# luchsonice/3dod

Measured on AMD Instinct MI355X. Metric: images/sec Cube R-CNN DLA34-FPN train step, higher is better.
Workload: dtype fp32; 1 GPU; Cube R-CNN DLA34+FPN train step (fwd+loss+bwd+allreduce+SGD), 4 img/GPU 512x512, Base_Omni3D.yaml semantics (BASELINE configs[3] per-GPU shard); global_batch=4, parallelism=dp1, weight_gradient_reduce=pixel splits stored and added in a fixed order (CR_DETERMINISTIC=1), valid=True

## Files before the change

3dod_amd/_lib.py:

```python
import ctypes
import os
import threading

import torch

_HERE = os.path.dirname(os.path.abspath(__file__))
LIB_PATH = os.path.join(_HERE, "lib", "libcr3dod.so")

c_void_p, c_int, c_int64, c_float = ctypes.c_void_p, ctypes.c_int, ctypes.c_int64, ctypes.c_float
P = c_void_p

SIGNATURES = {
    "cr_ctx_create": [c_int, P, ctypes.POINTER(P)],
    "cr_ctx_destroy": [P],
    "cr_ctx_set_stream": [P, P],
    "cr_abi_version": [],
    "cr_cuboid_corners": [P, P, P, c_int64, P],
    "cr_cubes_project_score": [P, P, c_int64, c_int64, P, c_int, c_float, c_float, P, P, P, P,
                               P, P, P, P, P, P, P, P, P],
    "cr_cubes_project_score_fast": [P, P, c_int64, c_int64, P, c_int, c_float, c_float, P, P, P, P,
                                    P, P, P, P, P, P, P, P, P, P],
    "cr_propose": [P, P, c_int64, P, c_int, c_int, P, P, P, c_int64, P, c_int, P, P, P, P, P],
    "cr_ransac_plane": [P, P, c_int64, P, c_int64, c_float, P, P, P],
    "cr_ransac_plane_batched": [P, P, P, c_int, c_int64, P, c_int64, c_float, P, P, P],
# ... 10 lines not shown
    "cr_scale_residual_layernorm": [P, P, P, P, P, P, P, P, c_int64, c_int, c_float],
    "cr_scale_residual": [P, P, P, P, P, c_int64, c_int],
    "cr_resize_bilinear_ac": [P, P, P, c_int, c_int, c_int, c_int, c_int, c_int],
    "cr_conv2d_fwd": [P, P, P, P, c_int, c_int, c_int, c_int, c_int, c_int, c_int, c_int, P, P, c_int, P, c_int, c_int, P],
    "cr_conv2d_bwd_data": [P, P, P, P, c_int, c_int, c_int, c_int, c_int, c_int, c_int, c_int, c_int, P, P],
    "cr_weight_split3": [P, P, P, c_int64, c_int],
    "cr_relu_bwd": [P, P, P, P, c_int64, c_int],
    "cr_gt_pack": [P, P, P, P, P, P, c_int, c_int, P, P, P, P],
    "cr_rpn_unpack": [P, P, P, c_int, c_int, c_int, c_int, P, P, P],
    "cr_rpn_pack_grad": [P, P, P, P, P, c_int, c_int, c_int, c_int],
    "cr_topk_blocks": [c_int64, c_int],
    "cr_topk": [P, P, c_int, c_int64, c_int, P, P, P],
    "cr_multi_seg": [P, P, c_int, c_int64, c_int],
    "cr_loss_guard": [P, P, c_int, c_float, P, P, P, c_int, c_float, c_float, P],
    "cr_step_counters": [P, P, P, P],
    "cr_weights_split3": [P, P, P, P, c_int, c_int64],
    "cr_conv2d_bwd_weight": [P, P, P, P, c_int, c_int, c_int, c_int, c_int, c_int, c_int, c_int, c_int, c_int],
    "cr_conv2d_bwd_weight_bias": [P, P, P, P, P, c_int, c_int, c_int, c_int, c_int, c_int, c_int, c_int, c_int, c_int],
    "cr_cast_f32_to_bf16": [P, P, P, c_int64],
    "cr_weight_transpose": [P, P, P, c_int, c_int, c_int, c_int],
    "cr_colsum_accum": [P, P, c_int, c_int64, c_int, P, P],
    "cr_bn_fwd": [P, P, P, c_int, P, P, P, P, c_int64, c_int, c_int, c_float, c_float, P, P, P, c_int],
    "cr_bn_bwd": [P, P, P, P, P, P, P, P, P, P, P, c_int64, c_int, c_int, c_int],
    "cr_bn_frozen_unfold": [P, P, P, P, P, P, P, c_float, P, c_int, P, P, c_int, c_int],
    "cr_pool2x_fwd": [P, P, P, c_int, c_int, c_int, c_int, c_int, c_int],
    "cr_pool2x_bwd": [P, P, P, P, c_int, c_int, c_int, c_int, c_int, c_int, P],
    "cr_upsample2x_add": [P, P, P, P, c_int, c_int, c_int, c_int, c_int],
    "cr_sum2x2": [P, P, P, c_int, c_int, c_int, c_int, c_int],
    "cr_preprocess": [P, P, P, c_int, c_int, c_int, P, P, c_int],
    "cr_roi_align_fwd": [P, P, P, P, P, c_int, c_int, P, c_int64, c_int, c_int, P, c_int],
    "cr_roi_align_bwd": [P, P, P, P, P, c_int, c_int, P, c_int64, c_int, c_int, P, c_int],
    "cr_conv2d_fwd_group": [P, c_int, P, P, P, P, P, P, c_int, c_int, c_int, c_int, P, P, c_int, c_int],
    "cr_wino_filter": [P, P, P, c_int, c_int, c_int],
    "cr_gemm_batched_f32": [P, P, P, P, c_int, c_int, c_int, c_int, c_int64, c_int64, c_int64],
    "cr_wino_input": [P, c_int, P, P, P, P, c_int, P, c_int64],
    "cr_wino_output": [P, c_int, P, P, P, P, P, c_int, c_int64, P, c_int, P],
    "cr_wino_dy": [P, c_int, P, P, P, P, c_int, P, c_int64, P],
    "cr_wino_filter_grad": [P, P, P, c_int, c_int, P, P],
    "cr_wgrad_batched_f32": [P, P, P, P, c_int, c_int, c_int, c_int, c_int64, c_int64, c_int64],
    "cr_conv2d_bwd_data_group": [P, c_int, P, P, P, P, P, P, c_int, c_int, c_int, c_int, c_int, P],
    "cr_conv2d_bwd_weight_group": [P, c_int, P, P, P, P, P, P, P, c_int, c_int, c_int, c_int, c_int],
    "cr_conv2d_bwd_weight_multi": [P, c_int, P, P, P, P, P, P, P, P, P, P, P, P, c_int],
    "cr_roi_align_bwd_set": [P, P, P, P, P, c_int, c_int, c_int, P, c_int64, c_int, c_int, P, c_int],
    "cr_nms_grouped": [P, P, P, c_int, c_int, c_float, P, P],
    "cr_cube_loss_fwd": [P, P, c_int64, c_int, c_int, c_int, c_int, P, P],
    "cr_cube_loss_bwd": [P, P, c_int64, c_int, c_int, c_int, c_int, P, P, P, P, P, P],
# ... 133 lines not shown
```

3dod_amd/csrc/conv.hip:

```cpp
#include "cr_common.h"
#include "cr_elem.h"
#include <stdlib.h>
#include <type_traits>

typedef __bf16 bf16x8 __attribute__((ext_vector_type(8)));
typedef __bf16 bf16x4 __attribute__((ext_vector_type(4)));
typedef short s16x4 __attribute__((ext_vector_type(4)));
typedef float f32x4 __attribute__((ext_vector_type(4)));

#define CONV_T 256

struct ConvP {
    const void* x;
    const void* w;
    void* y;
    const void* res;
    const float* bias;
    float* stats;
    int N, Hin, Win, Cin, Hout, Wout, Cout;
    int stride, pad, Kdim, M, cshift, relu;
    unsigned x_bytes, w_bytes;
    int f32;
    float* part;
    int ksplit, kstages;
// ... 3039 lines not shown

extern "C" int cr_fc_grad_accum(cr_ctx* ctx, const void* g, float* acc, int O, int C, int HW, int act_f32) {
    CR_CHECK_ARG(ctx && g && acc && O > 0 && C > 0 && HW > 0 && HW <= 1024, "cr_fc_grad_accum: bad args");
    if (HW == 1) {
        const int64_t n = (int64_t)O * C;
        CR_CHECK_ARG((((uintptr_t)g) & 7) == 0 && (((uintptr_t)acc) & 15) == 0, "cr_fc_grad_accum: misaligned");
        if (act_f32)
            hipLaunchKernelGGL(k_axpy_f32_f32, dim3((unsigned)cr_cdiv(cr_cdiv(n, 4), 256)), dim3(256), 0, ctx->stream,
                               (const float*)g, acc, n);
        else
            hipLaunchKernelGGL(k_axpy_bf16_f32, dim3((unsigned)cr_cdiv(cr_cdiv(n, 4), 256)), dim3(256), 0, ctx->stream,
                               (const u16*)g, acc, n);
    } else if (act_f32) {
        hipLaunchKernelGGL(k_fc_grad_accum<float>, dim3((unsigned)cr_cdiv(C, FC_CT), O), dim3(256),
                           FC_CT * (HW + 1) * sizeof(float), ctx->stream, (const float*)g, acc, C, HW);
    } else {
        hipLaunchKernelGGL(k_fc_grad_accum<u16>, dim3((unsigned)cr_cdiv(C, FC_CT), O), dim3(256),
                           FC_CT * (HW + 1) * sizeof(float), ctx->stream, (const u16*)g, acc, C, HW);
    }
    CR_LAUNCH_CHECK();
    return CR_OK;
}

__global__ __launch_bounds__(256) void k_bn_finalize(const float* __restrict__ stats, int nparts, int C, float count,
                                                     float eps, float momentum, float* __restrict__ mean_invstd,
                                                     float* __restrict__ running_mean, float* __restrict__ running_var) {
    __shared__ double ss[256], sq[256];
    const int c = blockIdx.x, t = threadIdx.x;
    double s = 0.0, q = 0.0;
    for (int r = t; r < nparts; r += 256) {
        s += (double)stats[(size_t)r * 2 * C + c];
        q += (double)stats[(size_t)r * 2 * C + C + c];
    }
    ss[t] = s; sq[t] = q;
    __syncthreads();
    for (int off = 128; off > 0; off >>= 1) {
        if (t < off) { ss[t] += ss[t + off]; sq[t] += sq[t + off]; }
        __syncthreads();
    }
    if (t == 0) {
        const double mean = ss[0] / (double)count;
        double var = sq[0] / (double)count - mean * mean;
        if (var < 0.0) var = 0.0;
        mean_invstd[c] = (float)mean;
        mean_invstd[C + c] = (float)(1.0 / sqrt(var + (double)eps));
        if (running_mean) {
            const double unbiased = count > 1.f ? var * (double)count / ((double)count - 1.0) : var;
            running_mean[c] = (float)((1.0 - momentum) * running_mean[c] + momentum * mean);
            running_var[c] = (float)((1.0 - momentum) * running_var[c] + momentum * unbiased);
        }
    }
}

template <typename T>
__global__ __launch_bounds__(256) void k_bn_apply(const T* __restrict__ x, const float* __restrict__ mean_invstd,
                                                  const float* __restrict__ gamma, const float* __restrict__ beta,
                                                  const T* __restrict__ res, T* __restrict__ y, int64_t M, int C,
                                                  int relu) {
    const int cg = C >> 3;
    const int64_t total = M * cg;
    for (int64_t i = (int64_t)blockIdx.x * blockDim.x + threadIdx.x; i < total; i += (int64_t)gridDim.x * blockDim.x) {
        const int c0 = (int)(i % cg) << 3;
        float xv[8], rv[8], o[8];
        load8<T>(x, (size_t)i * 8, xv);
        if (res) load8<T>(res, (size_t)i * 8, rv);
#pragma unroll
        for (int e = 0; e < 8; ++e) {
            const int c = c0 + e;
            float t = (xv[e] - mean_invstd[c]) * mean_invstd[C + c] * gamma[c] + beta[c];
            if (res) t += rv[e];
            o[e] = relu ? fmaxf(t, 0.f) : t;
        }
        store8<T>(y, (size_t)i * 8, o);
    }
}

template <typename T>
__global__ __launch_bounds__(256) void k_bn_apply_fused(const T* __restrict__ x, const float* __restrict__ stats, int nparts,
                                                        float count, float eps, float momentum, float* __restrict__ mean_invstd,
                                                        float* __restrict__ running_mean, float* __restrict__ running_var,
                                                        const float* __restrict__ gamma, const float* __restrict__ beta,
                                                        const T* __restrict__ res, T* __restrict__ y, int64_t M, int C, int relu,
                                                        int px_per_block) {
    __shared__ double sd[2][8][32];
    __shared__ float sc[2][32];
    const int t = threadIdx.x, ch = t & 31, rl = t >> 5;
    const int cbase = blockIdx.y * 32, c = cbase + ch;
    {
        double s = 0.0, q = 0.0;
        for (int r = rl; r < nparts; r += 8) {
            s += (double)stats[(size_t)r * 2 * C + c];
            q += (double)stats[(size_t)r * 2 * C + C + c];
// ... 17 lines not shown
            if (running_mean) {
                const double unbiased = count > 1.f ? var * (double)count / ((double)count - 1.0) : var;
                running_mean[cbase + t] = (float)((1.0 - momentum) * running_mean[cbase + t] + momentum * mean);
                running_var[cbase + t] = (float)((1.0 - momentum) * running_var[cbase + t] + momentum * unbiased);
            }
        }
    }
    __syncthreads();
    const int cgl = t & 3;
    float mu[8], is8[8], ga[8], be[8];
#pragma unroll
    for (int e = 0; e < 8; ++e) {
        mu[e] = sc[0][cgl * 8 + e]; is8[e] = sc[1][cgl * 8 + e];
        ga[e] = gamma[cbase + cgl * 8 + e]; be[e] = beta[cbase + cgl * 8 + e];
    }
    const int64_t m0 = (int64_t)blockIdx.x * px_per_block, m1 = m0 + px_per_block < M ? m0 + px_per_block : M;
    for (int64_t m = m0 + (t >> 2); m < m1; m += 64) {
        const size_t i8 = (size_t)m * C + cbase + cgl * 8;
        float xv[8], rv[8], o[8];
        load8<T>(x, i8, xv);
        if (res) load8<T>(res, i8, rv);
#pragma unroll
        for (int e = 0; e < 8; ++e) {
            float v = (xv[e] - mu[e]) * is8[e] * ga[e] + be[e];
            if (res) v += rv[e];
            o[e] = relu ? fmaxf(v, 0.f) : v;
        }
        store8<T>(y, i8, o);
    }
}

static constexpr int BN_FUSE_ROWS = 256;

extern "C" int cr_bn_fwd(cr_ctx* ctx, const void* x, const float* stats, int nparts, const float* gamma,
                         const float* beta, const void* residual, void* y, int64_t M, int C, int relu, float eps,
                         float momentum, float* mean_invstd, float* running_mean, float* running_var, int act_f32) {
    CR_CHECK_ARG(ctx && x && stats && gamma && beta && y && mean_invstd, "cr_bn_fwd: NULL pointer");
    CR_CHECK_ARG(M > 0 && C > 0 && C % 8 == 0 && nparts > 0, "cr_bn_fwd: bad dims M=%lld C=%d", (long long)M, C);
    if (C % 32 == 0 && nparts <= BN_FUSE_ROWS) {
        int64_t chunks = 1024 / (C / 32);
        if (chunks < 1) chunks = 1;
        int64_t ppb = cr_cdiv(M, chunks);
        ppb = (ppb + 63) / 64 * 64;
        const dim3 grid((unsigned)cr_cdiv(M, ppb), (unsigned)(C / 32));
        if (act_f32)
            hipLaunchKernelGGL(k_bn_apply_fused<float>, grid, dim3(256), 0, ctx->stream, (const float*)x, stats, nparts, (float)M,
                               eps, momentum, mean_invstd, running_mean, running_var, gamma, beta, (const float*)residual,
                               (float*)y, M, C, relu, (int)ppb);
        else
            hipLaunchKernelGGL(k_bn_apply_fused<u16>, grid, dim3(256), 0, ctx->stream, (const u16*)x, stats, nparts, (float)M,
                               eps, momentum, mean_invstd, running_mean, running_var, gamma, beta, (const u16*)residual,
                               (u16*)y, M, C, relu, (int)ppb);
        CR_LAUNCH_CHECK();
        return CR_OK;
    }
    hipLaunchKernelGGL(k_bn_finalize, dim3((unsigned)C), dim3(256), 0, ctx->stream, stats, nparts, C, (float)M, eps,
                       momentum, mean_invstd, running_mean, running_var);
    CR_LAUNCH_CHECK();
    const int64_t total = M * (C >> 3);
    const unsigned grid = (unsigned)(cr_cdiv(total, 256) < 4096 ? cr_cdiv(total, 256) : 4096);
    if (act_f32)
        hipLaunchKernelGGL(k_bn_apply<float>, dim3(grid), dim3(256), 0, ctx->stream, (const float*)x, mean_invstd, gamma, beta,
                           (const float*)residual, (float*)y, M, C, relu);
    else
        hipLaunchKernelGGL(k_bn_apply<u16>, dim3(grid), dim3(256), 0, ctx->stream, (const u16*)x, mean_invstd, gamma, beta,
                           (const u16*)residual, (u16*)y, M, C, relu);
    CR_LAUNCH_CHECK();
    return CR_OK;
}

#define BNB_MAXBLOCKS 1024
template <typename T>
__global__ __launch_bounds__(256) void k_bn_bwd_reduce(const T* __restrict__ dy, const T* __restrict__ out,
                                                       const T* __restrict__ x, const float* __restrict__ mean_invstd,
                                                       float* __restrict__ partial, int64_t M, int C, int relu) {
    extern __shared__ float s_acc[];
    const int cg = C >> 3;
    const int mycg = threadIdx.x % cg, myrow = threadIdx.x / cg;
    const int rows_per_block = blockDim.x / cg;
    const int c0 = mycg << 3;
    float a[8], b[8], mu[8], is[8];
#pragma unroll
    for (int e = 0; e < 8; ++e) { a[e] = 0.f; b[e] = 0.f; mu[e] = mean_invstd[c0 + e]; is[e] = mean_invstd[C + c0 + e]; }
    for (int64_t m = (int64_t)blockIdx.x * rows_per_block + myrow; m < M; m += (int64_t)gridDim.x * rows_per_block) {
        const size_t i8 = (size_t)(m * cg + mycg) * 8;
        float dv[8], xv[8], ov[8];
        load8<T>(dy, i8, dv);
        load8<T>(x, i8, xv);
        if (relu) load8<T>(out, i8, ov);
#pragma unroll
        for (int e = 0; e < 8; ++e) {
            const float gq = (!relu || ov[e] > 0.f) ? dv[e] : 0.f;
            const float xh = (xv[e] - mu[e]) * is[e];
            a[e] += gq;
            b[e] += gq * xh;
        }
    }
#pragma unroll
    for (int e = 0; e < 8; ++e) { s_acc[(myrow * 2 + 0) * C + c0 + e] = a[e]; s_acc[(myrow * 2 + 1) * C + c0 + e] = b[e]; }
    __syncthreads();
    float* dst = partial + (size_t)blockIdx.x * 2 * C;
    for (int i = threadIdx.x; i < 2 * C; i += blockDim.x) {
        const int which = i / C, c = i - which * C;
        float s = 0.f;
        for (int r = 0; r < rows_per_block; ++r) s += s_acc[(r * 2 + which) * C + c];
        dst[i] = s;
    }
}

__global__ __launch_bounds__(256) void k_bn_bwd_finalize(const float* __restrict__ partial, int nparts, int C,
                                                         float* __restrict__ sums, float* __restrict__ dgamma,
                                                         float* __restrict__ dbeta) {
    __shared__ double ss[256], sq[256];
    const int c = blockIdx.x, t = threadIdx.x;
    double s = 0.0, q = 0.0;
    for (int r = t; r < nparts; r += 256) {
        s += (double)partial[(size_t)r * 2 * C + c];
        q += (double)partial[(size_t)r * 2 * C + C + c];
    }
    ss[t] = s; sq[t] = q;
    __syncthreads();
    for (int off = 128; off > 0; off >>= 1) {
        if (t < off) { ss[t] += ss[t + off]; sq[t] += sq[t + off]; }
        __syncthreads();
    }
    if (t == 0) {
        sums[c] = (float)ss[0];
        sums[C + c] = (float)sq[0];
        dbeta[c] += (float)ss[0];
        dgamma[c] += (float)sq[0];
    }
}

template <typename T>
__global__ __launch_bounds__(256) void k_bn_bwd_apply(const T* __restrict__ dy, const T* __restrict__ out,
                                                      const T* __restrict__ x, const float* __restrict__ mean_invstd,
                                                      const float* __restrict__ gamma, const float* __restrict__ sums,
                                                      T* __restrict__ dx, T* __restrict__ dres, int64_t M, int C,
                                                      int relu) {
    const int cg = C >> 3;
    const float invM = 1.f / (float)M;
    const int64_t total = M * cg;
    for (int64_t i = (int64_t)blockIdx.x * blockDim.x + threadIdx.x; i < total; i += (int64_t)gridDim.x * blockDim.x) {
        const int c0 = (int)(i % cg) << 3;
        const size_t i8 = (size_t)i * 8;
        float dv[8], xv[8], ov[8], vd[8], vg[8];
        load8<T>(dy, i8, dv);
        load8<T>(x, i8, xv);
        if (relu) load8<T>(out, i8, ov);
#pragma unroll
        for (int e = 0; e < 8; ++e) {
            const int c = c0 + e;
            const float gq = (!relu || ov[e] > 0.f) ? dv[e] : 0.f;
            const float is = mean_invstd[C + c];
            const float xh = (xv[e] - mean_invstd[c]) * is;
            vd[e] = gamma[c] * is * (gq - sums[c] * invM - xh * sums[C + c] * invM);
            vg[e] = gq;
        }
        store8<T>(dx, i8, vd);
        if (dres) store8<T>(dres, i8, vg);
    }
}

template <typename T>
__global__ __launch_bounds__(256) void k_bn_bwd_apply_fused(const T* __restrict__ dy, const T* __restrict__ out,
                                                            const T* __restrict__ x, const float* __restrict__ mean_invstd,
                                                            const float* __restrict__ gamma, const float* __restrict__ partial,
                                                            int nparts, T* __restrict__ dx, T* __restrict__ dres,
                                                            float* __restrict__ dgamma, float* __restrict__ dbeta, int64_t M,
                                                            int C, int relu, int px_per_block) {
    __shared__ double sd[2][8][32];
    __shared__ float sc[4][32];
    const int t = threadIdx.x, ch = t & 31, rl = t >> 5;
    const int cbase = blockIdx.y * 32, c = cbase + ch;
    {
        double s = 0.0, q = 0.0;
        for (int r = rl; r < nparts; r += 8) {
            s += (double)partial[(size_t)r * 2 * C + c];
            q += (double)partial[(size_t)r * 2 * C + C + c];
        }
        sd[0][rl][ch] = s; sd[1][rl][ch] = q;
    }
    __syncthreads();
    if (t < 32) {
        double s = 0.0, q = 0.0;
#pragma unroll
        for (int r = 0; r < 8; ++r) { s += sd[0][r][t]; q += sd[1][r][t]; }
        const float sg = (float)s, sgx = (float)q, invM = 1.f / (float)M;
        const float is = mean_invstd[C + cbase + t];
        sc[0][t] = mean_invstd[cbase + t];
        sc[1][t] = is;
        sc[2][t] = sg * invM;
        sc[3][t] = sgx * invM;
        if (blockIdx.x == 0) { dbeta[cbase + t] += sg; dgamma[cbase + t] += sgx; }
    }
    __syncthreads();
    const int cgl = t & 3;
    float mu[8], is8[8], ga[8], k1[8], k2[8];
#pragma unroll
    for (int e = 0; e < 8; ++e) {
        const int cc = cgl * 8 + e;
        mu[e] = sc[0][cc]; is8[e] = sc[1][cc]; ga[e] = gamma[cbase + cc]; k1[e] = sc[2][cc]; k2[e] = sc[3][cc];
    }
    const int64_t m0 = (int64_t)blockIdx.x * px_per_block, m1 = m0 + px_per_block < M ? m0 + px_per_block : M;
    for (int64_t m = m0 + (t >> 2); m < m1; m += 64) {
        const size_t i8 = (size_t)m * C + cbase + cgl * 8;
        float dv[8], xv[8], ov[8], vd[8], vg[8];
        load8<T>(dy, i8, dv);
        load8<T>(x, i8, xv);
        if (relu) load8<T>(out, i8, ov);
#pragma unroll
        for (int e = 0; e < 8; ++e) {
            const float gq = (!relu || ov[e] > 0.f) ? dv[e] : 0.f;
            const float xh = (xv[e] - mu[e]) * is8[e];
            vd[e] = ga[e] * is8[e] * (gq - k1[e] - xh * k2[e]);
            vg[e] = gq;
        }
        store8<T>(dx, i8, vd);
        if (dres) store8<T>(dres, i8, vg);
    }
}

extern "C" int cr_bn_bwd(cr_ctx* ctx, const void* dy, const void* out, const void* x, const float* mean_invstd,
                         const float* gamma, float* sums, void* dx, void* dres, float* dgamma, float* dbeta,
                         int64_t M, int C, int relu, int act_f32) {
    CR_CHECK_ARG(ctx && dy && x && mean_invstd && gamma && sums && dx && dgamma && dbeta, "cr_bn_bwd: NULL pointer");
    CR_CHECK_ARG(!relu || out, "cr_bn_bwd: relu needs the forward output");
    CR_CHECK_ARG(M > 0 && C % 8 == 0 && C <= 2048 && 256 % (C >> 3) == 0, "cr_bn_bwd: unsupported C=%d", C);
    const int rows_per_block = 256 / (C >> 3);
    int64_t nb = cr_cdiv(M, (int64_t)rows_per_block * 8);
    if (nb > BNB_MAXBLOCKS) nb = BNB_MAXBLOCKS;
    if (nb < 1) nb = 1;
    float* reduced = sums + (size_t)BNB_MAXBLOCKS * 2 * C;
    const size_t shm = sizeof(float) * rows_per_block * 2 * C;
    if (act_f32)
        hipLaunchKernelGGL(k_bn_bwd_reduce<float>, dim3((unsigned)nb), dim3(256), shm, ctx->stream, (const float*)dy,
                           (const float*)out, (const float*)x, mean_invstd, sums, M, C, relu);
    else
        hipLaunchKernelGGL(k_bn_bwd_reduce<u16>, dim3((unsigned)nb), dim3(256), shm, ctx->stream, (const u16*)dy,
                           (const u16*)out, (const u16*)x, mean_invstd, sums, M, C, relu);
    CR_LAUNCH_CHECK();
    if (C % 32 == 0 && nb <= BN_FUSE_ROWS) {
        int64_t chunks = 1024 / (C / 32);
        if (chunks < 1) chunks = 1;
        int64_t ppb = cr_cdiv(M, chunks);
        ppb = (ppb + 63) / 64 * 64;
        const dim3 grid((unsigned)cr_cdiv(M, ppb), (unsigned)(C / 32));
        if (act_f32)
            hipLaunchKernelGGL(k_bn_bwd_apply_fused<float>, grid, dim3(256), 0, ctx->stream, (const float*)dy, (const float*)out,
                               (const float*)x, mean_invstd, gamma, sums, (int)nb, (float*)dx, (float*)dres, dgamma, dbeta, M, C,
                               relu, (int)ppb);
        else
            hipLaunchKernelGGL(k_bn_bwd_apply_fused<u16>, grid, dim3(256), 0, ctx->stream, (const u16*)dy, (const u16*)out,
                               (const u16*)x, mean_invstd, gamma, sums, (int)nb, (u16*)dx, (u16*)dres, dgamma, dbeta, M, C, relu,
                               (int)ppb);
        CR_LAUNCH_CHECK();
        return CR_OK;
    }
    hipLaunchKernelGGL(k_bn_bwd_finalize, dim3((unsigned)C), dim3(256), 0, ctx->stream, sums, (int)nb, C, reduced, dgamma,
                       dbeta);
    CR_LAUNCH_CHECK();
    const int64_t total = M * (C >> 3);
    const unsigned grid = (unsigned)(cr_cdiv(total, 256) < 4096 ? cr_cdiv(total, 256) : 4096);
    if (act_f32)
        hipLaunchKernelGGL(k_bn_bwd_apply<float>, dim3(grid), dim3(256), 0, ctx->stream, (const float*)dy, (const float*)out,
                           (const float*)x, mean_invstd, gamma, reduced, (float*)dx, (float*)dres, M, C, relu);
    else
        hipLaunchKernelGGL(k_bn_bwd_apply<u16>, dim3(grid), dim3(256), 0, ctx->stream, (const u16*)dy, (const u16*)out,
                           (const u16*)x, mean_invstd, gamma, reduced, (u16*)dx, (u16*)dres, M, C, relu);
    CR_LAUNCH_CHECK();
    return CR_OK;
}

template <typename T>
__global__ __launch_bounds__(256) void k_colsum_partial(const T* __restrict__ x, int64_t M, int C, int rows_per_block,
                                                        float* __restrict__ partial) {
    const int64_t r0 = (int64_t)blockIdx.x * rows_per_block;
    const int64_t r1 = r0 + rows_per_block < M ? r0 + rows_per_block : M;
    for (int c = threadIdx.x; c < C; c += 256) {
        float s = 0.f;
        for (int64_t r = r0; r < r1; ++r) {
            if (sizeof(T) == 2) s += bf2f(((const u16*)x)[r * C + c]);
            else s += ((const float*)x)[r * C + c];
        }
        partial[(size_t)blockIdx.x * C + c] = s;
    }
}

__global__ __launch_bounds__(256) void k_colsum_final(const float* __restrict__ partial, int nparts, int C,
                                                      float* __restrict__ out) {
    __shared__ double ss[256];
    const int c = blockIdx.x, t = threadIdx.x;
    double s = 0.0;
    for (int r = t; r < nparts; r += 256) s += (double)partial[(size_t)r * C + c];
// ... 399 lines not shown
```

3dod_amd/csrc/cr_elem.h:

```cpp
#pragma once
#include <hip/hip_runtime.h>

typedef unsigned short u16;

__device__ __forceinline__ float bf2f(u16 b) { return __uint_as_float(((unsigned)b) << 16); }
__device__ __forceinline__ u16 f2bf(float f) {
    __bf16 b = (__bf16)f;
    return __builtin_bit_cast(u16, b);
}

__device__ __forceinline__ void unpack8(const uint4 v, float* f) {
    f[0] = bf2f((u16)(v.x & 0xffff)); f[1] = bf2f((u16)(v.x >> 16));
    f[2] = bf2f((u16)(v.y & 0xffff)); f[3] = bf2f((u16)(v.y >> 16));
    f[4] = bf2f((u16)(v.z & 0xffff)); f[5] = bf2f((u16)(v.z >> 16));
    f[6] = bf2f((u16)(v.w & 0xffff)); f[7] = bf2f((u16)(v.w >> 16));
}
__device__ __forceinline__ uint4 pack8(const float* f) {
    uint4 o;
    o.x = (unsigned)f2bf(f[0]) | ((unsigned)f2bf(f[1]) << 16);
    o.y = (unsigned)f2bf(f[2]) | ((unsigned)f2bf(f[3]) << 16);
    o.z = (unsigned)f2bf(f[4]) | ((unsigned)f2bf(f[5]) << 16);
    o.w = (unsigned)f2bf(f[6]) | ((unsigned)f2bf(f[7]) << 16);
    return o;
}

template <typename T> __device__ __forceinline__ void load8(const T* __restrict__ p, size_t e, float* f);
template <> __device__ __forceinline__ void load8<u16>(const u16* __restrict__ p, size_t e, float* f) {
    unpack8(*reinterpret_cast<const uint4*>(p + e), f);
}
template <> __device__ __forceinline__ void load8<float>(const float* __restrict__ p, size_t e, float* f) {
    const float4 a = *reinterpret_cast<const float4*>(p + e), b = *reinterpret_cast<const float4*>(p + e + 4);
    f[0] = a.x; f[1] = a.y; f[2] = a.z; f[3] = a.w; f[4] = b.x; f[5] = b.y; f[6] = b.z; f[7] = b.w;
}
template <typename T> __device__ __forceinline__ void store8(T* __restrict__ p, size_t e, const float* f);
template <> __device__ __forceinline__ void store8<u16>(u16* __restrict__ p, size_t e, const float* f) {
    *reinterpret_cast<uint4*>(p + e) = pack8(f);
}
template <> __device__ __forceinline__ void store8<float>(float* __restrict__ p, size_t e, const float* f) {
    *reinterpret_cast<float4*>(p + e) = make_float4(f[0], f[1], f[2], f[3]);
    *reinterpret_cast<float4*>(p + e + 4) = make_float4(f[4], f[5], f[6], f[7]);
}
template <typename T> __device__ __forceinline__ float load1(const T* __restrict__ p, size_t e);
template <> __device__ __forceinline__ float load1<u16>(const u16* __restrict__ p, size_t e) { return bf2f(p[e]); }
template <> __device__ __forceinline__ float load1<float>(const float* __restrict__ p, size_t e) { return p[e]; }
```

3dod_amd/hipops.py:

```python
import contextlib
import ctypes
import os

import torch

from . import _lib

bf16 = torch.bfloat16
f32 = torch.float32
STAT_REPL = 32

_PRECISIONS = {"fp32": (f32, 1), "f32": (f32, 1), "float32": (f32, 1), "fp32x3": (f32, 2), "bf16": (bf16, 0),
               "bfloat16": (bf16, 0)}
_ACT = [_PRECISIONS[os.environ.get("CR_PRECISION", "fp32").lower()]]


def set_precision(name):
    prev = precision()
    _ACT[0] = _PRECISIONS[str(name).lower()]
    return prev


def precision():
    return {0: "bf16", 1: "fp32", 2: "fp32x3"}[_ACT[0][1]]
# ... 307 lines not shown
            nparts = (M + 63) // 64
            stats = torch.empty((nparts, 2, Cout), dtype=f32, device=dev)
            y_raw = conv_fwd_raw(x, wb, Cout, k, stride, pad, stats=stats)
            out = torch.empty_like(y_raw)
            mi = torch.empty((2, Cout), dtype=f32, device=dev)
            _lib.call("cr_bn_fwd", y_raw, stats, nparts, gamma.detach(), beta.detach(), residual, out, M, Cout, int(relu),
                      float(eps), float(momentum), mi, running_mean, running_var, af)
        else:
            K_ = weight.numel() // Cout
            wf32 = torch.empty((Cout, K_), dtype=f32, device=dev)
            bias_f = torch.empty((Cout,), dtype=f32, device=dev)
            _lib.call("cr_fold_bn", weight.detach(), gamma.detach(), beta.detach(), running_mean, running_var, float(eps), wf32,
                      bias_f, Cout, K_, 1)
            if x.dtype == bf16:
                wf = torch.empty((Cout, K_), dtype=bf16, device=dev)
                _lib.call("cr_cast_f32_to_bf16", wf32, wf, wf32.numel())
            else:
                wf = wf32
            out = conv_fwd_raw(x, wf, Cout, k, stride, pad, bias=bias_f, residual=residual, relu=relu)
            y_raw, mi = wf32, None
            ctx.frozen = (running_mean, running_var, float(eps))
        ctx.cfg = (k, stride, pad, relu, training, residual is not None)
        ctx.beta_ref = beta
        ctx.save_for_backward(x, weight, gamma, y_raw, out if relu else None, mi)
        return out

    @staticmethod
    def backward(ctx, dout):
        return _ConvBN._backward_impl(ctx, dout)

    @staticmethod
    def _backward_impl(ctx, dout, want_dx=None, want_dw=None):
        x, weight, gamma, y_raw, out, mi = ctx.saved_tensors
        k, stride, pad, relu, training, has_res = ctx.cfg
        root = want_dx is not None
        need_dx = ctx.needs_input_grad[0] if want_dx is None else want_dx
        need_dw = ctx.needs_input_grad[1] if want_dw is None else want_dw
        if not training:
            return _ConvBN._frozen_backward(ctx, dout, need_dx, need_dw, root)
        Cout = weight.shape[0]
        dev = x.device
        dout = dout.to(x.dtype).contiguous()
        M = y_raw.numel() // Cout
        sums = torch.empty((1025, 2, Cout), dtype=f32, device=dev)
        dx_raw = torch.empty_like(y_raw)
        dres = torch.empty_like(y_raw) if has_res else None
        gs, bs = grad_sink(gamma), grad_sink(ctx.beta_ref)
        if gs is not None and bs is not None:
            dgamma, dbeta, ret_g, ret_b = gs, bs, None, None
        else:
            dgamma = torch.zeros((Cout,), dtype=f32, device=dev)
            dbeta = torch.zeros((Cout,), dtype=f32, device=dev)
            ret_g, ret_b = dgamma, dbeta
        _lib.call("cr_bn_bwd", dout, out, y_raw, mi, gamma.detach(), sums, dx_raw, dres, dgamma, dbeta, M, Cout, int(relu),
                  _af(x))
        (xslot, xi), (rslot, ri) = ctx.slots
        if rslot is not None and dres is not None:
            _slot_put(rslot, dres)
            dres = None
        dx = None
        if need_dx:
            _, wt = prepared_weights(weight, True, x.dtype)
            if xslot is not None and xi > 1:
                _slot_put(xslot, conv_bwd_data_raw(dx_raw, wt, x.shape, k, stride, pad, accumulate=_slot_fold(xslot)))
            else:
                acc = _slot_take(xslot) if xslot is not None else None
                dx = conv_bwd_data_raw(dx_raw, wt, x.shape, k, stride, pad, accumulate=acc)
        elif xslot is not None:
            raise RuntimeError("gradient slot registered for an input that needs no gradient")
        dw = conv_bwd_weight_raw(dx_raw, x, k, stride, pad, grad_sink(weight)) if need_dw else None
        if root:
            return dx_raw, dw, ret_g, ret_b
        return dx, dw, ret_g, ret_b, dres, None, None, None, None, None, None, None, None, None

    @staticmethod
    def _frozen_backward(ctx, dout, need_dx, need_dw, root):
        x, weight, gamma, wf32, out, _ = ctx.saved_tensors
        k, stride, pad, relu, _, has_res = ctx.cfg
# ... 1701 lines not shown
```

include/cr3dod.h:

```cpp
#ifndef CR3DOD_H
#define CR3DOD_H

#include <stdint.h>

#ifdef __cplusplus
extern "C" {
#endif

typedef struct cr_ctx cr_ctx;

#define CR_OK 0
#define CR_EINVAL (-22)
#define CR_ENOMEM (-12)
#define CR_EHIP (-5)
#define CR_ERANGE (-34)

int cr_ctx_create(int device, void* hip_stream, cr_ctx** out);
int cr_ctx_destroy(cr_ctx* ctx);
int cr_ctx_set_stream(cr_ctx* ctx, void* hip_stream);
const char* cr_last_error(void);
int cr_abi_version(void);


int cr_cuboid_corners(cr_ctx* ctx, const float* box6, const float* R, int64_t n, float* verts);
// ... 99 lines not shown

int cr_conv2d_fwd_group(cr_ctx* ctx, int n, const void* const* xs, const void* const* ws, void* const* ys, const int* Ns,
                        const int* Hs, const int* Ws, int Cin, int Cout, int ks, int pad, const float* const* biases,
                        const void* const* residuals, int relu, int act_f32);
int cr_conv2d_bwd_data_group(cr_ctx* ctx, int n, const void* const* dys, const void* const* wts, void* const* dxs,
                             const int* Ns, const int* Hs, const int* Ws, int Cin, int Cout, int ks, int pad, int act_f32,
                             const void* const* accumulates);
int cr_conv2d_bwd_weight_group(cr_ctx* ctx, int n, const void* const* dys, const void* const* xs, float* const* dws,
                               float* const* dbiases, const int* Ns, const int* Hs, const int* Ws, int Cin, int Cout, int ks,
                               int pad, int act_f32);
int cr_conv2d_bwd_weight_multi(cr_ctx* ctx, int n, const void* const* dys, const void* const* xs, float* const* dws,
                               float* const* dbiases, const int* Ns, const int* Hs, const int* Ws, const int* Cins,
                               const int* Couts, const int* kss, const int* strides, const int* pads, int act_f32);
int cr_cast_f32_to_bf16(cr_ctx* ctx, const float* src, void* dst, int64_t n);
int cr_colsum_accum(cr_ctx* ctx, const void* x, int is_f32, int64_t M, int C, float* ws, float* out);
int cr_weight_transpose(cr_ctx* ctx, const float* w, void* wt, int Cout, int ks, int Cin, int act_f32);

int cr_bn_fwd(cr_ctx* ctx, const void* x, const float* stats, int nparts, const float* gamma, const float* beta,
              const void* residual, void* y, int64_t M, int C, int relu, float eps, float momentum,
              float* mean_invstd, float* running_mean, float* running_var, int act_f32);
int cr_bn_bwd(cr_ctx* ctx, const void* dy, const void* out, const void* x, const float* mean_invstd,
              const float* gamma, float* sums, void* dx, void* dres, float* dgamma, float* dbeta, int64_t M,
              int C, int relu, int act_f32);
int cr_bn_frozen_unfold(cr_ctx* ctx, const float* dwf, const float* sg, const float* w, const float* gamma,
                        const float* mean, const float* var, float eps, float* dw, int accumulate, float* dgamma,
                        float* dbeta, int Cout, int K);

int cr_pool2x_fwd(cr_ctx* ctx, const void* x, void* y, int N, int H, int W, int C, int window, int act_f32);
int cr_pool2x_bwd(cr_ctx* ctx, const void* x, const void* dy, void* dx, int N, int H, int W, int C, int window, int act_f32,
                  const void* accumulate);
int cr_upsample2x_add(cr_ctx* ctx, const void* lat, const void* top, void* y, int N, int H, int W, int C, int act_f32);
int cr_sum2x2(cr_ctx* ctx, const void* dy, void* dtop, int N, int H, int W, int C, int act_f32);
int cr_preprocess(cr_ctx* ctx, const unsigned char* img, void* y, int N, int H, int W, const float* mean3,
                  const float* std3, int act_f32);

int cr_roi_align_fwd(cr_ctx* ctx, const void* const* feats, const int* Hs, const int* Ws, const float* scales,
                     int nlev, int C, const float* rois, int64_t R, int PH, int PW, void* out, int act_f32);
int cr_roi_align_bwd(cr_ctx* ctx, float* const* grads, const int* Hs, const int* Ws, const float* scales,
                     int nlev, int C, const float* rois, int64_t R, int PH, int PW, const void* dout, int act_f32);
int cr_roi_align_bwd_set(cr_ctx* ctx, float* const* grads, const int* Hs, const int* Ws, const float* scales,
                         int nlev, int C, int N, const float* rois, int64_t R, int PH, int PW, const void* dout,
                         int act_f32);
int cr_nms_grouped(cr_ctx* ctx, const float* boxes, const int* counts, int G, int maxn, float thresh,
                   void* mask_ws, unsigned char* keep);

int cr_cube_loss_fwd(cr_ctx* ctx, const float* const* inputs, int64_t n, int allocentric, int chamfer_pose,
// ... 130 lines not shown
```

Measured before the change: 279.3 images/s.

## Recompute BN ReLU mask in backward and parallelize BN stats finalize

```diff
diff --git a/3dod_amd/_lib.py b/3dod_amd/_lib.py
--- a/3dod_amd/_lib.py
+++ b/3dod_amd/_lib.py
@@ -56,6 +56,7 @@
     "cr_colsum_accum": [P, P, c_int, c_int64, c_int, P, P],
     "cr_bn_fwd": [P, P, P, c_int, P, P, P, P, c_int64, c_int, c_int, c_float, c_float, P, P, P, c_int],
     "cr_bn_bwd": [P, P, P, P, P, P, P, P, P, P, P, c_int64, c_int, c_int, c_int],
+    "cr_bn_bwd_mask": [P, P, P, P, P, P, P, P, P, P, P, P, c_int64, c_int, c_int, c_int],
     "cr_bn_frozen_unfold": [P, P, P, P, P, P, P, c_float, P, c_int, P, P, c_int, c_int],
     "cr_pool2x_fwd": [P, P, P, c_int, c_int, c_int, c_int, c_int, c_int],
     "cr_pool2x_bwd": [P, P, P, P, c_int, c_int, c_int, c_int, c_int, c_int, P],
diff --git a/3dod_amd/csrc/conv.hip b/3dod_amd/csrc/conv.hip
--- a/3dod_amd/csrc/conv.hip
+++ b/3dod_amd/csrc/conv.hip
@@ -3085,35 +3085,81 @@
     return CR_OK;
 }
 
+__device__ __forceinline__ void bn_finalize_tail(double s, double q, int c, int C, float count, float eps, float momentum,
+                                                 float* __restrict__ mean_invstd, float* __restrict__ running_mean,
+                                                 float* __restrict__ running_var) {
+    __shared__ double ss[256], sq[256];
+    const int t = threadIdx.x;
+    ss[t] = s; sq[t] = q;
+    __syncthreads();
+    for (int off = 128; off > 0; off >>= 1) {
+        if (t < off) { ss[t] += ss[t + off]; sq[t] += sq[t + off]; }
+        __syncthreads();
+    }
+    if (t == 0) {
+#pragma clang fp contract(off)
+        const double mean = ss[0] / (double)count;
+        double var = __builtin_fma(-mean, mean, sq[0] / (double)count);
+        if (var < 0.0) var = 0.0;
+        mean_invstd[c] = (float)mean;
+        mean_invstd[C + c] = (float)(1.0 / sqrt(var + (double)eps));
+        if (running_mean) {
+            const double unbiased = count > 1.f ? var * (double)count / ((double)count - 1.0) : var;
+            running_mean[c] = (float)__builtin_fma((double)momentum, mean, (1.0 - momentum) * running_mean[c]);
+            running_var[c] = (float)__builtin_fma((double)momentum, unbiased, (1.0 - momentum) * running_var[c]);
+        }
+    }
+}
+
 __global__ __launch_bounds__(256) void k_bn_finalize(const float* __restrict__ stats, int nparts, int C, float count,
                                                      float eps, float momentum, float* __restrict__ mean_invstd,
                                                      float* __restrict__ running_mean, float* __restrict__ running_var) {
-    __shared__ double ss[256], sq[256];
     const int c = blockIdx.x, t = threadIdx.x;
     double s = 0.0, q = 0.0;
     for (int r = t; r < nparts; r += 256) {
         s += (double)stats[(size_t)r * 2 * C + c];
         q += (double)stats[(size_t)r * 2 * C + C + c];
     }
-    ss[t] = s; sq[t] = q;
-    __syncthreads();
-    for (int off = 128; off > 0; off >>= 1) {
-        if (t < off) { ss[t] += ss[t + off]; sq[t] += sq[t + off]; }
-        __syncthreads();
-    }
-    if (t == 0) {
-        const double mean = ss[0] / (double)count;
-        double var = sq[0] / (double)count - mean * mean;
-        if (var < 0.0) var = 0.0;
-        mean_invstd[c] = (float)mean;
-        mean_invstd[C + c] = (float)(1.0 / sqrt(var + (double)eps));
-        if (running_mean) {
-            const double unbiased = count > 1.f ? var * (double)count / ((double)count - 1.0) : var;
-            running_mean[c] = (float)((1.0 - momentum) * running_mean[c] + momentum * mean);
-            running_var[c] = (float)((1.0 - momentum) * running_var[c] + momentum * unbiased);
-        }
-    }
-}
+    bn_finalize_tail(s, q, c, C, count, eps, momentum, mean_invstd, running_mean, running_var);
+}
+
+static constexpr int BN_LANE_BATCH = 8;
+__global__ __launch_bounds__(256) void k_bn_stats_lanes(const float* __restrict__ stats, int nparts, int C2,
+                                                        double* __restrict__ lanes) {
+    const int f = blockIdx.x * 256 + threadIdx.x;
+    const int t = f / C2, j = f - t * C2;
+    const float* p = stats + (size_t)t * C2 + j;
+    const size_t step = (size_t)256 * C2;
+    double s = 0.0;
+    int r = t;
+    for (; r + 256 * (BN_LANE_BATCH - 1) < nparts; r += 256 * BN_LANE_BATCH) {
+        float v[BN_LANE_BATCH];
+#pragma unroll
+        for (int u = 0; u < BN_LANE_BATCH; ++u) v[u] = p[(size_t)u * step];
+#pragma unroll
+        for (int u = 0; u < BN_LANE_BATCH; ++u) s += (double)v[u];
+        p += BN_LANE_BATCH * step;
+    }
+    for (; r < nparts; r += 256) { s += (double)*p; p += step; }
+    lanes[f] = s;
+}
+
+__global__ __launch_bounds__(256) void k_bn_finalize_lanes(const double* __restrict__ lanes, int C, float count, float eps,
+                                                           float momentum, float* __restrict__ mean_invstd,
+                                                           float* __restrict__ running_mean, float* __restrict__ running_var) {
+    const int c = blockIdx.x, t = threadIdx.x;
+    bn_finalize_tail(lanes[(size_t)t * 2 * C + c], lanes[(size_t)t * 2 * C + C + c], c, C, count, eps, momentum, mean_invstd,
+                     running_mean, running_var);
+}
+
+__device__ __forceinline__ float bn_affine(float x, float mean, float invstd, float gamma, float beta) {
+#pragma clang fp contract(off)
+    const float xh = (x - mean) * invstd;
+    return __builtin_fmaf(xh, gamma, beta);
+}
+template <typename T> __device__ __forceinline__ bool bn_relu_on(float v);
+template <> __device__ __forceinline__ bool bn_relu_on<float>(float v) { return fmaxf(v, 0.f) > 0.f; }
+template <> __device__ __forceinline__ bool bn_relu_on<u16>(float v) { return bf2f(f2bf(fmaxf(v, 0.f))) > 0.f; }
 
 template <typename T>
 __global__ __launch_bounds__(256) void k_bn_apply(const T* __restrict__ x, const float* __restrict__ mean_invstd,
@@ -3130,7 +3176,7 @@
 #pragma unroll
         for (int e = 0; e < 8; ++e) {
             const int c = c0 + e;
-            float t = (xv[e] - mean_invstd[c]) * mean_invstd[C + c] * gamma[c] + beta[c];
+            float t = bn_affine(xv[e], mean_invstd[c], mean_invstd[C + c], gamma[c], beta[c]);
             if (res) t += rv[e];
             o[e] = relu ? fmaxf(t, 0.f) : t;
         }
@@ -3194,7 +3240,7 @@
         if (res) load8<T>(res, i8, rv);
 #pragma unroll
         for (int e = 0; e < 8; ++e) {
-            float v = (xv[e] - mu[e]) * is8[e] * ga[e] + be[e];
+            float v = bn_affine(xv[e], mu[e], is8[e], ga[e], be[e]);
             if (res) v += rv[e];
             o[e] = relu ? fmaxf(v, 0.f) : v;
         }
@@ -3203,6 +3249,7 @@
 }
 
 static constexpr int BN_FUSE_ROWS = 256;
+static constexpr int BN_LANES_MIN_ROWS = 2048;
 
 extern "C" int cr_bn_fwd(cr_ctx* ctx, const void* x, const float* stats, int nparts, const float* gamma,
                          const float* beta, const void* residual, void* y, int64_t M, int C, int relu, float eps,
@@ -3226,8 +3273,17 @@
         CR_LAUNCH_CHECK();
         return CR_OK;
     }
-    hipLaunchKernelGGL(k_bn_finalize, dim3((unsigned)C), dim3(256), 0, ctx->stream, stats, nparts, C, (float)M, eps,
-                       momentum, mean_invstd, running_mean, running_var);
+    const size_t lanes_bytes = sizeof(double) * 256 * 2 * C;
+    if (nparts >= BN_LANES_MIN_ROWS && ctx->ws && lanes_bytes <= ctx->ws_bytes) {
+        double* lanes = (double*)ctx->ws;
+        hipLaunchKernelGGL(k_bn_stats_lanes, dim3((unsigned)(2 * C)), dim3(256), 0, ctx->stream, stats, nparts, 2 * C, lanes);
+        CR_LAUNCH_CHECK();
+        hipLaunchKernelGGL(k_bn_finalize_lanes, dim3((unsigned)C), dim3(256), 0, ctx->stream, lanes, C, (float)M, eps,
+                           momentum, mean_invstd, running_mean, running_var);
+    } else {
+        hipLaunchKernelGGL(k_bn_finalize, dim3((unsigned)C), dim3(256), 0, ctx->stream, stats, nparts, C, (float)M, eps,
+                           momentum, mean_invstd, running_mean, running_var);
+    }
     CR_LAUNCH_CHECK();
     const int64_t total = M * (C >> 3);
     const unsigned grid = (unsigned)(cr_cdiv(total, 256) < 4096 ? cr_cdiv(total, 256) : 4096);
@@ -3242,34 +3298,45 @@
 }
 
 #define BNB_MAXBLOCKS 1024
-template <typename T>
-__global__ __launch_bounds__(256) void k_bn_bwd_reduce(const T* __restrict__ dy, const T* __restrict__ out,
+#define BNB_V (MASKX ? 4 : 8)
+#define BNB_VSHIFT (MASKX ? 2 : 3)
+template <typename T, bool MASKX>
+__global__ __launch_bounds__(MASKX ? 512 : 256) void k_bn_bwd_reduce(const T* __restrict__ dy, const T* __restrict__ out,
                                                        const T* __restrict__ x, const float* __restrict__ mean_invstd,
+                                                       const float* __restrict__ gamma, const float* __restrict__ beta,
                                                        float* __restrict__ partial, int64_t M, int C, int relu) {
     extern __shared__ float s_acc[];
-    const int cg = C >> 3;
+    constexpr int V = BNB_V;
+    const int cg = C >> BNB_VSHIFT;
     const int mycg = threadIdx.x % cg, myrow = threadIdx.x / cg;
     const int rows_per_block = blockDim.x / cg;
-    const int c0 = mycg << 3;
-    float a[8], b[8], mu[8], is[8];
-#pragma unroll
-    for (int e = 0; e < 8; ++e) { a[e] = 0.f; b[e] = 0.f; mu[e] = mean_invstd[c0 + e]; is[e] = mean_invstd[C + c0 + e]; }
+    const int c0 = mycg << BNB_VSHIFT;
+    float a[V], b[V], mu[V], is[V];
+#pragma unroll
+    for (int e = 0; e < V; ++e) { a[e] = 0.f; b[e] = 0.f; mu[e] = mean_invstd[c0 + e]; is[e] = mean_invstd[C + c0 + e]; }
+    float ga[V], be[V];
+    if (MASKX) {
+#pragma unroll
+        for (int e = 0; e < V; ++e) { ga[e] = gamma[c0 + e]; be[e] = beta[c0 + e]; }
+    }
     for (int64_t m = (int64_t)blockIdx.x * rows_per_block + myrow; m < M; m += (int64_t)gridDim.x * rows_per_block) {
-        const size_t i8 = (size_t)(m * cg + mycg) * 8;
-        float dv[8], xv[8], ov[8];
-        load8<T>(dy, i8, dv);
-        load8<T>(x, i8, xv);
-        if (relu) load8<T>(out, i8, ov);
-#pragma unroll
-        for (int e = 0; e < 8; ++e) {
-            const float gq = (!relu || ov[e] > 0.f) ? dv[e] : 0.f;
+        const size_t i8 = (size_t)(m * cg + mycg) * V;
+        float dv[V], xv[V], ov[V];
+        loadv<T, V>(dy, i8, dv);
+        loadv<T, V>(x, i8, xv);
+        if (relu && !MASKX) loadv<T, V>(out, i8, ov);
+#pragma unroll
+        for (int e = 0; e < V; ++e) {
+            const bool on = MASKX ? bn_relu_on<T>(bn_affine(xv[e], mu[e], is[e], ga[e], be[e]))
+                                  : (!relu || ov[e] > 0.f);
+            const float gq = on ? dv[e] : 0.f;
             const float xh = (xv[e] - mu[e]) * is[e];
             a[e] += gq;
             b[e] += gq * xh;
         }
     }
 #pragma unroll
-    for (int e = 0; e < 8; ++e) { s_acc[(myrow * 2 + 0) * C + c0 + e] = a[e]; s_acc[(myrow * 2 + 1) * C + c0 + e] = b[e]; }
+    for (int e = 0; e < V; ++e) { s_acc[(myrow * 2 + 0) * C + c0 + e] = a[e]; s_acc[(myrow * 2 + 1) * C + c0 + e] = b[e]; }
     __syncthreads();
     float* dst = partial + (size_t)blockIdx.x * 2 * C;
     for (int i = threadIdx.x; i < 2 * C; i += blockDim.x) {
@@ -3304,41 +3371,44 @@
     }
 }
 
-template <typename T>
+template <typename T, bool MASKX>
 __global__ __launch_bounds__(256) void k_bn_bwd_apply(const T* __restrict__ dy, const T* __restrict__ out,
                                                       const T* __restrict__ x, const float* __restrict__ mean_invstd,
-                                                      const float* __restrict__ gamma, const float* __restrict__ sums,
-                                                      T* __restrict__ dx, T* __restrict__ dres, int64_t M, int C,
-                                                      int relu) {
-    const int cg = C >> 3;
+                                                      const float* __restrict__ gamma, const float* __restrict__ beta,
+                                                      const float* __restrict__ sums, T* __restrict__ dx,
+                                                      T* __restrict__ dres, int64_t M, int C, int relu) {
+    constexpr int V = BNB_V;
+    const int cg = C >> BNB_VSHIFT;
     const float invM = 1.f / (float)M;
     const int64_t total = M * cg;
     for (int64_t i = (int64_t)blockIdx.x * blockDim.x + threadIdx.x; i < total; i += (int64_t)gridDim.x * blockDim.x) {
-        const int c0 = (int)(i % cg) << 3;
-        const size_t i8 = (size_t)i * 8;
-        float dv[8], xv[8], ov[8], vd[8], vg[8];
-        load8<T>(dy, i8, dv);
-        load8<T>(x, i8, xv);
-        if (relu) load8<T>(out, i8, ov);
-#pragma unroll
-        for (int e = 0; e < 8; ++e) {
+        const int c0 = (int)(i % cg) << BNB_VSHIFT;
+        const size_t i8 = (size_t)i * V;
+        float dv[V], xv[V], ov[V], vd[V], vg[V];
+        loadv<T, V>(dy, i8, dv);
+        loadv<T, V>(x, i8, xv);
+        if (relu && !MASKX) loadv<T, V>(out, i8, ov);
+#pragma unroll
+        for (int e = 0; e < V; ++e) {
             const int c = c0 + e;
-            const float gq = (!relu || ov[e] > 0.f) ? dv[e] : 0.f;
             const float is = mean_invstd[C + c];
+            const bool on = MASKX ? bn_relu_on<T>(bn_affine(xv[e], mean_invstd[c], is, gamma[c], beta[c])) : (!relu || ov[e] > 0.f);
+            const float gq = on ? dv[e] : 0.f;
             const float xh = (xv[e] - mean_invstd[c]) * is;
             vd[e] = gamma[c] * is * (gq - sums[c] * invM - xh * sums[C + c] * invM);
             vg[e] = gq;
         }
-        store8<T>(dx, i8, vd);
-        if (dres) store8<T>(dres, i8, vg);
-    }
-}
-
-template <typename T>
+        storev<T, V>(dx, i8, vd);
+        if (dres) storev<T, V>(dres, i8, vg);
+    }
+}
+
+template <typename T, bool MASKX>
 __global__ __launch_bounds__(256) void k_bn_bwd_apply_fused(const T* __restrict__ dy, const T* __restrict__ out,
                                                             const T* __restrict__ x, const float* __restrict__ mean_invstd,
-                                                            const float* __restrict__ gamma, const float* __restrict__ partial,
-                                                            int nparts, T* __restrict__ dx, T* __restrict__ dres,
+                                                            const float* __restrict__ gamma, const float* __restrict__ beta,
+                                                            const float* __restrict__ partial, int nparts,
+                                                            T* __restrict__ dx, T* __restrict__ dres,
                                                             float* __restrict__ dgamma, float* __restrict__ dbeta, int64_t M,
                                                             int C, int relu, int px_per_block) {
     __shared__ double sd[2][8][32];
@@ -3367,50 +3437,48 @@
         if (blockIdx.x == 0) { dbeta[cbase + t] += sg; dgamma[cbase + t] += sgx; }
     }
     __syncthreads();
-    const int cgl = t & 3;
-    float mu[8], is8[8], ga[8], k1[8], k2[8];
-#pragma unroll
-    for (int e = 0; e < 8; ++e) {
-        const int cc = cgl * 8 + e;
+    constexpr int V = BNB_V, G = 32 / V;
+    const int cgl = t & (G - 1);
+    float mu[V], is8[V], ga[V], be[V], k1[V], k2[V];
+#pragma unroll
+    for (int e = 0; e < V; ++e) {
+        const int cc = cgl * V + e;
         mu[e] = sc[0][cc]; is8[e] = sc[1][cc]; ga[e] = gamma[cbase + cc]; k1[e] = sc[2][cc]; k2[e] = sc[3][cc];
+        be[e] = MASKX ? beta[cbase + cc] : 0.f;
     }
     const int64_t m0 = (int64_t)blockIdx.x * px_per_block, m1 = m0 + px_per_block < M ? m0 + px_per_block : M;
-    for (int64_t m = m0 + (t >> 2); m < m1; m += 64) {
-        const size_t i8 = (size_t)m * C + cbase + cgl * 8;
-        float dv[8], xv[8], ov[8], vd[8], vg[8];
-        load8<T>(dy, i8, dv);
-        load8<T>(x, i8, xv);
-        if (relu) load8<T>(out, i8, ov);
-#pragma unroll
-        for (int e = 0; e < 8; ++e) {
-            const float gq = (!relu || ov[e] > 0.f) ? dv[e] : 0.f;
+    for (int64_t m = m0 + t / G; m < m1; m += 256 / G) {
+        const size_t i8 = (size_t)m * C + cbase + cgl * V;
+        float dv[V], xv[V], ov[V], vd[V], vg[V];
+        loadv<T, V>(dy, i8, dv);
+        loadv<T, V>(x, i8, xv);
+        if (relu && !MASKX) loadv<T, V>(out, i8, ov);
+#pragma unroll
+        for (int e = 0; e < V; ++e) {
+            const bool on = MASKX ? bn_relu_on<T>(bn_affine(xv[e], mu[e], is8[e], ga[e], be[e]))
+                                  : (!relu || ov[e] > 0.f);
+            const float gq = on ? dv[e] : 0.f;
             const float xh = (xv[e] - mu[e]) * is8[e];
             vd[e] = ga[e] * is8[e] * (gq - k1[e] - xh * k2[e]);
             vg[e] = gq;
         }
-        store8<T>(dx, i8, vd);
-        if (dres) store8<T>(dres, i8, vg);
-    }
-}
-
-extern "C" int cr_bn_bwd(cr_ctx* ctx, const void* dy, const void* out, const void* x, const float* mean_invstd,
-                         const float* gamma, float* sums, void* dx, void* dres, float* dgamma, float* dbeta,
-                         int64_t M, int C, int relu, int act_f32) {
-    CR_CHECK_ARG(ctx && dy && x && mean_invstd && gamma && sums && dx && dgamma && dbeta, "cr_bn_bwd: NULL pointer");
-    CR_CHECK_ARG(!relu || out, "cr_bn_bwd: relu needs the forward output");
-    CR_CHECK_ARG(M > 0 && C % 8 == 0 && C <= 2048 && 256 % (C >> 3) == 0, "cr_bn_bwd: unsupported C=%d", C);
+        storev<T, V>(dx, i8, vd);
+        if (dres) storev<T, V>(dres, i8, vg);
+    }
+}
+
+template <typename T, bool MASKX>
+static int bn_bwd_launch(cr_ctx* ctx, const T* dy, const T* out, const T* x, const float* mean_invstd, const float* gamma,
+                         const float* beta, float* sums, T* dx, T* dres, float* dgamma, float* dbeta, int64_t M, int C,
+                         int relu) {
     const int rows_per_block = 256 / (C >> 3);
     int64_t nb = cr_cdiv(M, (int64_t)rows_per_block * 8);
     if (nb > BNB_MAXBLOCKS) nb = BNB_MAXBLOCKS;
     if (nb < 1) nb = 1;
     float* reduced = sums + (size_t)BNB_MAXBLOCKS * 2 * C;
     const size_t shm = sizeof(float) * rows_per_block * 2 * C;
-    if (act_f32)
-        hipLaunchKernelGGL(k_bn_bwd_reduce<float>, dim3((unsigned)nb), dim3(256), shm, ctx->stream, (const float*)dy,
-                           (const float*)out, (const float*)x, mean_invstd, sums, M, C, relu);
-    else
-        hipLaunchKernelGGL(k_bn_bwd_reduce<u16>, dim3((unsigned)nb), dim3(256), shm, ctx->stream, (const u16*)dy,
-                           (const u16*)out, (const u16*)x, mean_invstd, sums, M, C, relu);
+    hipLaunchKernelGGL((k_bn_bwd_reduce<T, MASKX>), dim3((unsigned)nb), dim3(MASKX ? 512 : 256), shm, ctx->stream, dy, out, x, mean_invstd,
+                       gamma, beta, sums, M, C, relu);
     CR_LAUNCH_CHECK();
     if (C % 32 == 0 && nb <= BN_FUSE_ROWS) {
         int64_t chunks = 1024 / (C / 32);
@@ -3418,30 +3486,50 @@
         int64_t ppb = cr_cdiv(M, chunks);
         ppb = (ppb + 63) / 64 * 64;
         const dim3 grid((unsigned)cr_cdiv(M, ppb), (unsigned)(C / 32));
-        if (act_f32)
-            hipLaunchKernelGGL(k_bn_bwd_apply_fused<float>, grid, dim3(256), 0, ctx->stream, (const float*)dy, (const float*)out,
-                               (const float*)x, mean_invstd, gamma, sums, (int)nb, (float*)dx, (float*)dres, dgamma, dbeta, M, C,
-                               relu, (int)ppb);
-        else
-            hipLaunchKernelGGL(k_bn_bwd_apply_fused<u16>, grid, dim3(256), 0, ctx->stream, (const u16*)dy, (const u16*)out,
-                               (const u16*)x, mean_invstd, gamma, sums, (int)nb, (u16*)dx, (u16*)dres, dgamma, dbeta, M, C, relu,
-                               (int)ppb);
+        hipLaunchKernelGGL((k_bn_bwd_apply_fused<T, MASKX>), grid, dim3(256), 0, ctx->stream, dy, out, x, mean_invstd, gamma,
+                           beta, sums, (int)nb, dx, dres, dgamma, dbeta, M, C, relu, (int)ppb);
         CR_LAUNCH_CHECK();
         return CR_OK;
     }
     hipLaunchKernelGGL(k_bn_bwd_finalize, dim3((unsigned)C), dim3(256), 0, ctx->stream, sums, (int)nb, C, reduced, dgamma,
                        dbeta);
     CR_LAUNCH_CHECK();
-    const int64_t total = M * (C >> 3);
-    const unsigned grid = (unsigned)(cr_cdiv(total, 256) < 4096 ? cr_cdiv(total, 256) : 4096);
-    if (act_f32)
-        hipLaunchKernelGGL(k_bn_bwd_apply<float>, dim3(grid), dim3(256), 0, ctx->stream, (const float*)dy, (const float*)out,
-                           (const float*)x, mean_invstd, gamma, reduced, (float*)dx, (float*)dres, M, C, relu);
-    else
-        hipLaunchKernelGGL(k_bn_bwd_apply<u16>, dim3(grid), dim3(256), 0, ctx->stream, (const u16*)dy, (const u16*)out,
-                           (const u16*)x, mean_invstd, gamma, reduced, (u16*)dx, (u16*)dres, M, C, relu);
+    const int64_t total = M * (C >> BNB_VSHIFT);
+    const int64_t cap = MASKX ? 8192 : 4096;
+    const unsigned grid = (unsigned)(cr_cdiv(total, 256) < cap ? cr_cdiv(total, 256) : cap);
+    hipLaunchKernelGGL((k_bn_bwd_apply<T, MASKX>), dim3(grid), dim3(256), 0, ctx->stream, dy, out, x, mean_invstd, gamma, beta,
+                       reduced, dx, dres, M, C, relu);
     CR_LAUNCH_CHECK();
     return CR_OK;
+}
+
+extern "C" int cr_bn_bwd(cr_ctx* ctx, const void* dy, const void* out, const void* x, const float* mean_invstd,
+                         const float* gamma, float* sums, void* dx, void* dres, float* dgamma, float* dbeta,
+                         int64_t M, int C, int relu, int act_f32) {
+    CR_CHECK_ARG(ctx && dy && x && mean_invstd && gamma && sums && dx && dgamma && dbeta, "cr_bn_bwd: NULL pointer");
+    CR_CHECK_ARG(!relu || out, "cr_bn_bwd: relu needs the forward output");
+    CR_CHECK_ARG(M > 0 && C % 8 == 0 && C <= 2048 && 256 % (C >> 3) == 0, "cr_bn_bwd: unsupported C=%d", C);
+    if (act_f32)
+        return bn_bwd_launch<float, false>(ctx, (const float*)dy, (const float*)out, (const float*)x, mean_invstd, gamma, nullptr,
+                                           sums, (float*)dx, (float*)dres, dgamma, dbeta, M, C, relu);
+    return bn_bwd_launch<u16, false>(ctx, (const u16*)dy, (const u16*)out, (const u16*)x, mean_invstd, gamma, nullptr, sums,
+                                     (u16*)dx, (u16*)dres, dgamma, dbeta, M, C, relu);
+}
+
+extern "C" int cr_bn_bwd_mask(cr_ctx* ctx, const void* dy, const void* out, const void* x, const float* mean_invstd,
+                              const float* gamma, const float* beta, float* sums, void* dx, void* dres, float* dgamma,
+                              float* dbeta, int64_t M, int C, int relu, int act_f32) {
+    CR_CHECK_ARG(ctx && dy && x && mean_invstd && gamma && beta && sums && dx && dgamma && dbeta, "cr_bn_bwd_mask: NULL pointer");
+    CR_CHECK_ARG(!relu || out || !dres, "cr_bn_bwd_mask: a residual layer's relu needs the forward output");
+    CR_CHECK_ARG(M > 0 && C % 8 == 0 && C <= 2048 && 256 % (C >> 3) == 0, "cr_bn_bwd_mask: unsupported C=%d", C);
+    if (relu && !out) {
+        if (act_f32)
+            return bn_bwd_launch<float, true>(ctx, (const float*)dy, nullptr, (const float*)x, mean_invstd, gamma, beta, sums,
+                                              (float*)dx, nullptr, dgamma, dbeta, M, C, relu);
+        return bn_bwd_launch<u16, true>(ctx, (const u16*)dy, nullptr, (const u16*)x, mean_invstd, gamma, beta, sums, (u16*)dx,
+                                        nullptr, dgamma, dbeta, M, C, relu);
+    }
+    return cr_bn_bwd(ctx, dy, out, x, mean_invstd, gamma, sums, dx, dres, dgamma, dbeta, M, C, relu, act_f32);
 }
 
 template <typename T>
diff --git a/3dod_amd/csrc/cr_elem.h b/3dod_amd/csrc/cr_elem.h
--- a/3dod_amd/csrc/cr_elem.h
+++ b/3dod_amd/csrc/cr_elem.h
@@ -40,6 +40,32 @@
     *reinterpret_cast<float4*>(p + e) = make_float4(f[0], f[1], f[2], f[3]);
     *reinterpret_cast<float4*>(p + e + 4) = make_float4(f[4], f[5], f[6], f[7]);
 }
+template <typename T> __device__ __forceinline__ void load4(const T* __restrict__ p, size_t e, float* f);
+template <> __device__ __forceinline__ void load4<u16>(const u16* __restrict__ p, size_t e, float* f) {
+    const uint2 v = *reinterpret_cast<const uint2*>(p + e);
+    f[0] = bf2f((u16)(v.x & 0xffff)); f[1] = bf2f((u16)(v.x >> 16));
+    f[2] = bf2f((u16)(v.y & 0xffff)); f[3] = bf2f((u16)(v.y >> 16));
+}
+template <> __device__ __forceinline__ void load4<float>(const float* __restrict__ p, size_t e, float* f) {
+    const float4 a = *reinterpret_cast<const float4*>(p + e);
+    f[0] = a.x; f[1] = a.y; f[2] = a.z; f[3] = a.w;
+}
+template <typename T> __device__ __forceinline__ void store4(T* __restrict__ p, size_t e, const float* f);
+template <> __device__ __forceinline__ void store4<u16>(u16* __restrict__ p, size_t e, const float* f) {
+    uint2 o;
+    o.x = (unsigned)f2bf(f[0]) | ((unsigned)f2bf(f[1]) << 16);
+    o.y = (unsigned)f2bf(f[2]) | ((unsigned)f2bf(f[3]) << 16);
+    *reinterpret_cast<uint2*>(p + e) = o;
+}
+template <> __device__ __forceinline__ void store4<float>(float* __restrict__ p, size_t e, const float* f) {
+    *reinterpret_cast<float4*>(p + e) = make_float4(f[0], f[1], f[2], f[3]);
+}
+template <typename T, int V> __device__ __forceinline__ void loadv(const T* __restrict__ p, size_t e, float* f) {
+    if (V == 8) load8<T>(p, e, f); else load4<T>(p, e, f);
+}
+template <typename T, int V> __device__ __forceinline__ void storev(T* __restrict__ p, size_t e, const float* f) {
+    if (V == 8) store8<T>(p, e, f); else store4<T>(p, e, f);
+}
 template <typename T> __device__ __forceinline__ float load1(const T* __restrict__ p, size_t e);
 template <> __device__ __forceinline__ float load1<u16>(const u16* __restrict__ p, size_t e) { return bf2f(p[e]); }
 template <> __device__ __forceinline__ float load1<float>(const float* __restrict__ p, size_t e) { return p[e]; }
diff --git a/3dod_amd/hipops.py b/3dod_amd/hipops.py
--- a/3dod_amd/hipops.py
+++ b/3dod_amd/hipops.py
@@ -353,7 +353,8 @@
             ctx.frozen = (running_mean, running_var, float(eps))
         ctx.cfg = (k, stride, pad, relu, training, residual is not None)
         ctx.beta_ref = beta
-        ctx.save_for_backward(x, weight, gamma, y_raw, out if relu else None, mi)
+        keep_out = relu and not (training and residual is None)
+        ctx.save_for_backward(x, weight, gamma, y_raw, out if keep_out else None, mi)
         return out
 
     @staticmethod
@@ -383,8 +384,12 @@
             dgamma = torch.zeros((Cout,), dtype=f32, device=dev)
             dbeta = torch.zeros((Cout,), dtype=f32, device=dev)
             ret_g, ret_b = dgamma, dbeta
-        _lib.call("cr_bn_bwd", dout, out, y_raw, mi, gamma.detach(), sums, dx_raw, dres, dgamma, dbeta, M, Cout, int(relu),
-                  _af(x))
+        if relu and not has_res:
+            _lib.call("cr_bn_bwd_mask", dout, None, y_raw, mi, gamma.detach(), ctx.beta_ref.detach(), sums, dx_raw, None, dgamma,
+                      dbeta, M, Cout, 1, _af(x))
+        else:
+            _lib.call("cr_bn_bwd", dout, out, y_raw, mi, gamma.detach(), sums, dx_raw, dres, dgamma, dbeta, M, Cout, int(relu),
+                      _af(x))
         (xslot, xi), (rslot, ri) = ctx.slots
         if rslot is not None and dres is not None:
             _slot_put(rslot, dres)
diff --git a/include/cr3dod.h b/include/cr3dod.h
--- a/include/cr3dod.h
+++ b/include/cr3dod.h
@@ -145,6 +145,9 @@
 int cr_bn_bwd(cr_ctx* ctx, const void* dy, const void* out, const void* x, const float* mean_invstd,
               const float* gamma, float* sums, void* dx, void* dres, float* dgamma, float* dbeta, int64_t M,
               int C, int relu, int act_f32);
+int cr_bn_bwd_mask(cr_ctx* ctx, const void* dy, const void* out, const void* x, const float* mean_invstd,
+                   const float* gamma, const float* beta, float* sums, void* dx, void* dres, float* dgamma,
+                   float* dbeta, int64_t M, int C, int relu, int act_f32);
 int cr_bn_frozen_unfold(cr_ctx* ctx, const float* dwf, const float* sg, const float* w, const float* gamma,
                         const float* mean, const float* var, float eps, float* dw, int accumulate, float* dgamma,
                         float* dbeta, int Cout, int K);
```

After: 282.2 images/s (median of 6 runs). +1.1%, better.
